# Cyan4973/FiniteStateEntropy

Measured on AMD Instinct MI355X. Metric: MB/s encode+decode per GPU on 32KB probagen blocks; bit-exact vs CPU ref, higher is better.
Workload: dtype u8; 1 GPU; probagen Proba14, 100000 x 32KB blocks per GPU, FSE encode+decode (one-shot calls at the reference's default limits: tableLog 11, decode maxLog 12), bit-exact check; blocks_per_gpu=100000, block_bytes=32768, codec=fse, parity=fse: roundtrip-all-blocks

## Files before the change

finitestateentropy_amd/csrc/fse_tables.hip:

```cpp
#include "internal.h"

#include "wave_glue.h"
#include "ncount_reader.h"
#include "fse_wave_build.h"

template <u32 MAXC>
DEV void fse_wave_build_ctable(const WaveBuildLds& w, const int nn[4], u32 maxSV, u32 tl, u32* img, u32 lane)
{
    u16* const cumAll = w.cumP;
    *(uint2*)(w.nrm + 4 * lane) = make_uint2(((u32)nn[0] & 0xFFFFu) | ((u32)nn[1] << 16), ((u32)nn[2] & 0xFFFFu) | ((u32)nn[3] << 16));
    __syncthreads();
    const u32 ts = 1u << tl;
    u16* const stateTable = (u16*)(img + 1);
    u32* const tt = img + 1 + (ts >> 1);
    {
        u32 eff[4], laneSum = 0;
#pragma unroll
        for (int i = 0; i < 4; ++i) { eff[i] = nn[i] == -1 ? 1u : (u32)nn[i]; laneSum += eff[i]; }
        u32 total;
        u32 run = wb_scan_excl(laneSum, lane, &total);
#pragma unroll
        for (int i = 0; i < 4; ++i) {
            const u32 s = 4 * lane + i;
            cumAll[s] = (u16)run;
            if (s <= maxSV) {
                if (nn[i] == 0) { tt[2 * s] = 0; tt[2 * s + 1] = ((tl + 1) << 16) - ts; }
                else if (nn[i] == -1 || nn[i] == 1) { tt[2 * s] = run - 1u; tt[2 * s + 1] = (tl << 16) - ts; }
                else {
                    const u32 maxBitsOut = tl - hibit32((u32)nn[i] - 1);
                    tt[2 * s] = run - (u32)nn[i];
                    tt[2 * s + 1] = (maxBitsOut << 16) - ((u32)nn[i] << maxBitsOut);
                }
            }
            run += eff[i];
        }
        if (lane == 0) img[0] = tl | (maxSV << 16);
    }
    __syncthreads();
    wave_spread_rank<MAXC>(w, maxSV, tl, lane, [&](u32 s) { return (u32)cumAll[s]; },
                     [&](u32 u, u32 s, u32 r, u32 first) { (void)s; stateTable[first + r] = (u16)(ts + u); });
}

template <u32 MAXC>
__global__ __launch_bounds__(64) void k_fse_cprep(FseCPrepArgs a, u32 capTs)
{
    extern __shared__ __attribute__((aligned(16))) u8 wbLds[];
    const size_t b = blockIdx.x;
    const u32 lane = threadIdx.x;
    const size_t n = view_size(a.src, b);
    FseMeta m; m.state = 0; m.hdrSize = 0; m.tableLog = 0; m.maxSV = 0; m.pace = 0;
    const size_t top = a.histResults[b];
    size_t result = 0; bool go = false;
    if (n <= 1) result = 0;
    else if (is_err(top)) result = top;
    else if (top == n) result = 1;
    else if (top == 1 || top < (n >> 7)) result = 0;
    else go = true;
    const WaveBuildLds w = wave_build_carve(wbLds, capTs, true);
    u32* const hdrImg = w.cnt;
    u32 maxSV = 0, tl = 0;
    int nn[4] = { 0, 0, 0, 0 };
    if (go) {
        maxSV = a.maxSVs[b];
        tl = wg_optimal_tablelog(a.tableLogReq, n, maxSV, 2);
        if ((1u << tl) > 64u * MAXC || (1u << tl) > capTs) { result = FERR(tableLog_tooLarge); go = false; }
    }
    if (go) {
        const uint4 cv = ((const uint4*)(a.counts + b * 256))[lane];
        const u32 c[4] = { cv.x, cv.y, cv.z, cv.w };
        for (u32 i = lane; i < 136; i += 64) hdrImg[i] = 0;
        const size_t e = wg_normalize<64>(nn, c, (u64)n, maxSV, tl, lane);
        if (is_err(e)) { result = e; go = false; }
    }
    __syncthreads();
    if (go) {
        const size_t h = wg_write_ncount<64>(hdrImg, a.dstCapacity, nn, maxSV, tl, lane);
        if (is_err(h)) { result = h; go = false; }
        else m.hdrSize = (u32)h;
    }
    __syncthreads();
    if (!go) { if (lane == 0) { a.meta[b] = m; a.results[b] = result; } return; }
    {   u8* const dst = a.dst + b * a.dstStride;
        const u8* const hb = (const u8*)hdrImg;
        for (u32 i = lane; i < m.hdrSize; i += 64) dst[i] = hb[i];
    }
    int top1 = nn[0] > nn[1] ? nn[0] : nn[1]; top1 = nn[2] > top1 ? nn[2] : top1; top1 = nn[3] > top1 ? nn[3] : top1;
    top1 = wave_max_i32(top1);
    m.state = ((u32)top1 * 64u > (63u << tl) || n < FSE_ENC_WAVE_MIN) ? FSE_ENC_LANE : FSE_ENC_PAR;
    {
        u32 present = (nn[0] != 0) + (nn[1] != 0) + (nn[2] != 0) + (nn[3] != 0);
        present = wg_sum<64>(present);
        const u32 mix = (1u << tl) / (present ? present : 1u);
        m.pace = mix < 64u ? 0u : mix < 128u ? 1u : mix < 256u ? 2u : 3u;
    }
    m.tableLog = tl; m.maxSV = maxSV;
    if (lane == 0) a.meta[b] = m;
    fse_wave_build_ctable<MAXC>(w, nn, maxSV, tl, a.ctables + b * a.ctStrideU32, lane);
}

__global__ __launch_bounds__(64) void k_fse_dparse(FseDPrepArgs a)
{
    __shared__ __attribute__((aligned(16))) u32 stage[NCS_WORDS];
    const size_t b0 = (size_t)blockIdx.x * 64, b = b0 + threadIdx.x;
    const u32 lane = threadIdx.x;
    const bool have = b < a.nBlocks;
    const u8* const in = have ? view_ptr(a.csrc, b) : nullptr;
    const size_t cSize = have ? view_size(a.csrc, b) : 0;
    bool done = false;
    if (have && a.rawRle) { const size_t orig = a.origSizes ? a.origSizes[b] : a.uniformOrig; done = cSize == orig || cSize == 1; }
    const u32 staged = ncount_stage(stage, in, cSize, lane, have && !done);
    {   uint4* const rows = (uint4*)(a.norms + b0 * 256);
        const u32 nRows = a.nBlocks - b0 < 64 ? (u32)(a.nBlocks - b0) : 64u;
        for (u32 i = lane; i < nRows * 32u; i += 64) rows[i] = make_uint4(0, 0, 0, 0);
    }
    __syncthreads();
    int cls = -1;
    if (have) {
        FseMeta m; m.state = 0; m.hdrSize = 0; m.tableLog = 0; m.maxSV = 0; m.pace = 0; m.pace = 0;
        size_t result = 0;
        if (!done) do {
            u32 tl = 0, maxSV = 255;
            s16* const norm = a.norms + b * 256;
            const size_t h = ncount_read_staged(norm, &maxSV, &tl, stage + lane, staged, in, cSize);
            if (is_err(h)) { result = h; break; }
            if (tl > a.maxLog) { result = FERR(tableLog_tooLarge); break; }
            cls = FSE_DCLS_REV11;
            if (tl > FSE_DEC_FAST_MAXLOG) {
                int top = 0;
                for (u32 i = 0; i <= maxSV >> 3; ++i) {
                    const uint4 v = ((const uint4*)norm)[i];
                    const u32 q[4] = { v.x, v.y, v.z, v.w };
#pragma unroll
                    for (int k = 0; k < 4; ++k) { const int lo = (s16)(q[k] & 0xFFFFu), hi = (s16)(q[k] >> 16); top = lo > top ? lo : top; top = hi > top ? hi : top; }
                }
                cls = 2 * top > (1 << tl) ? FSE_DCLS_PLAIN : FSE_DCLS_REV12;
            }
            m.state = 1u | ((u32)cls << 2); m.hdrSize = (u32)h; m.tableLog = tl; m.maxSV = maxSV;
        } while (0);
        a.meta[b] = m;
        if (m.state == 0 && !done) a.results[b] = result;
    }
    if (cls >= 0) { const size_t bin = view_size(a.csrc, b) >> FSE_DBIN_LOG; cls = cls * FSE_DBINS + (int)(bin < FSE_DBINS - 1 ? bin : FSE_DBINS - 1); }
    const unsigned long long below = (1ull << lane) - 1ull;
    unsigned long long todo = __ballot(cls >= 0);
    while (todo) {
        const int leader = __builtin_ctzll(todo);
        const int c = __shfl(cls, leader, WAVE);
        const unsigned long long mask = __ballot(cls == c);
        u32 base = 0;
        if ((int)lane == leader) {
            base = atomicAdd(&a.counts[c], (u32)__builtin_popcountll(mask));
            atomicAdd(&a.counts[FSE_DCLS_COUNT + c / FSE_DBINS], (u32)__builtin_popcountll(mask));
        }
        base = (u32)__shfl((int)base, leader, WAVE);
        if (cls == c) a.lists[(size_t)c * a.nBlocks + base + (u32)__builtin_popcountll(mask & below)] = (u32)b;
        todo &= ~mask;
    }
}

template <u32 MAXC>
__global__ __launch_bounds__(64) void k_fse_dbuild(FseDPrepArgs a, u32 capTs, int firstList, int nLists, u32 ldsCapTs)
{
    extern __shared__ __attribute__((aligned(16))) u8 wbLds[];
    {   u32 total = 0;
        for (int k = firstList / (int)FSE_DBINS; k < (firstList + nLists) / (int)FSE_DBINS; ++k) total += a.counts[FSE_DCLS_COUNT + k];
        if (blockIdx.x >= total) return;
    }
    constexpr int MAXL = 2 * FSE_DBINS;
    static_assert(FSE_DBINS % 4 == 0, "the list lengths are read as 16-byte vectors");
    uint4 cv[MAXL / 4];
#pragma unroll
    for (int i = 0; i < MAXL / 4; ++i) cv[i] = 4 * i < nLists ? ((const uint4*)(a.counts + firstList))[i] : make_uint4(0, 0, 0, 0);
    u32 idx = blockIdx.x;
    int c = firstList + nLists;
    {   u32 before = 0; bool found = false;
#pragma unroll
        for (int i = 0; i < MAXL; ++i) {
            const uint4 v = cv[i >> 2];
            const u32 n = (i & 3) == 0 ? v.x : (i & 3) == 1 ? v.y : (i & 3) == 2 ? v.z : v.w;
            const bool here = !found & (i < nLists) & (idx < before + n);
            c = here ? firstList + i : c; idx = here ? idx - before : idx;
            found |= here;
            before += n;
        }
    }
    if (c == firstList + nLists) return;
    const size_t b = a.lists[(size_t)c * a.nBlocks + idx];
    const u32 lane = threadIdx.x;
    const FseMeta m = a.meta[b];
    if (m.state == 0) return;
    const u32 tl = m.tableLog, ts = 1u << tl;
    if (ts > ldsCapTs || ts > 64u * MAXC) {
        if (lane == 0) { a.meta[b].state = 0; a.results[b] = FERR(tableLog_tooLarge); }
        return;
    }
    const WaveBuildLds w = wave_build_carve(wbLds, ldsCapTs, false);
    *(uint2*)(w.nrm + 4 * lane) = *(const uint2*)(a.norms + b * 256 + 4 * lane);
    __syncthreads();
    const bool rev = ((m.state >> 2) & 3u) != FSE_DCLS_PLAIN;
    u16* const A = a.atab + b * capTs;
    u8* const S = a.symtab + b * capTs;
    const bool fast = wave_spread_rank<MAXC>(w, m.maxSV, tl, lane, [&](u32 s) { return (u32)(int)w.nrm[s]; }, [&](u32 u, u32 s, u32 r, u32 nrm) {
        const int n = (int)nrm;
        const u32 next = (n > 0 ? (u32)n : 1u) + r;
        const u32 nb = tl - hibit32(next);
        const u32 ns = (next << nb) - ts;
        const u32 x = rev ? __brev(u) >> (32u - tl) : u;
        A[x] = rev ? (u16)(nb | ((__brev(ns) >> (32u - tl)) << 5)) : (u16)((ns & 0xFFFu) | (nb << 12));
        S[x] = (u8)s;
    });
    if (lane == 0) a.meta[b].state = m.state | (fast ? 2u : 0u);
}

__global__ __launch_bounds__(256) void k_fse_export_dtable(FseDPrepArgs a, u32 capTs, u32* dtables, size_t dtStrideU32)
{
    const size_t b = blockIdx.x;
    const FseMeta m = a.meta[b];
    if (m.state == 0) return;
    const u32 tl = m.tableLog, ts = 1u << tl;
    const bool rev = ((m.state >> 2) & 3u) != FSE_DCLS_PLAIN;
    const u16* const A = a.atab + b * capTs;
    const u8* const S = a.symtab + b * capTs;
    u32* const dt = dtables + b * dtStrideU32;
    if (threadIdx.x == 0) dt[0] = tl | ((m.state & 2u) ? 1u << 16 : 0u);
    for (u32 x = threadIdx.x; x < ts; x += blockDim.x) {
        const u32 i = rev ? __brev(x) >> (32u - tl) : x;
        const u32 c = A[i];
        const u32 nb = rev ? (c & 31u) : (c >> 12);
        const u32 ns = rev ? __brev(c >> 5) >> (32u - tl) : (c & 0xFFFu);
        dt[1 + x] = ns | ((u32)S[i] << 16) | (nb << 24);
    }
}
hipError_t launch_fse_export_dtables(const FseDPrepArgs& a, u32* dtables, size_t dtStrideU32, hipStream_t s)
{
    if (a.nBlocks == 0) return hipSuccess;
    hipLaunchKernelGGL(k_fse_export_dtable, dim3((unsigned)a.nBlocks), dim3(256), 0, s, a, 1u << a.maxLog, dtables, dtStrideU32);
    return hipGetLastError();
}

DEV size_t fse_norm_load_checked(int nn[4], const s16* nb, u32 maxSV, u32 tl, u32 maxTl, u32 lane)
{
    if (maxSV > 255u) return FERR(maxSymbolValue_tooLarge);
    if (tl > maxTl) return FERR(tableLog_tooLarge);
    if (tl == 0 || tl == 1 || tl == 3) return FERR(GENERIC);
    u32 cells = 0; bool bad = false;
#pragma unroll
    for (int i = 0; i < 4; ++i) {
        nn[i] = 4 * lane + i <= maxSV ? (int)nb[4 * lane + i] : 0;
        bad |= nn[i] < -1;
        cells += nn[i] == -1 ? 1u : nn[i] > 0 ? (u32)nn[i] : 0u;
    }
    cells = wg_sum<64>(cells);
    return (wg_any<64>(bad, lane) || cells != (1u << tl)) ? FERR(GENERIC) : 0;
}
template <u32 MAXC>
__global__ __launch_bounds__(64) void k_fse_ctable_from_norm(const s16* norms, size_t normStride, const u32* maxSVs, u32 tl, u32* ctables, size_t ctStrideU32,
                                                            size_t* results, u32 capTs)
{
    extern __shared__ __attribute__((aligned(16))) u8 wbLds[];
    const size_t b = blockIdx.x;
    const u32 lane = threadIdx.x;
    const u32 maxSV = maxSVs[b];
    int nn[4] = { 0, 0, 0, 0 };
    static_assert(MAXC == 32 || MAXC == 64, "64 * MAXC cells = a table of tableLog 11 or 12");
    const size_t r = fse_norm_load_checked(nn, norms + b * normStride, maxSV, tl, MAXC == 32 ? 11u : FSE_MAX_TL, lane);
    if (lane == 0) results[b] = r;
    if (is_err(r)) return;
    fse_wave_build_ctable<MAXC>(wave_build_carve(wbLds, capTs, true), nn, maxSV, tl, ctables + b * ctStrideU32, lane);
}
hipError_t launch_fse_ctable_from_norm(const s16* norms, size_t normStride, const u32* maxSVs, u32 tl, u32* ctables, size_t ctStrideU32, size_t* results,
                                       size_t nBlocks, hipStream_t s)
{
    if (nBlocks == 0) return hipSuccess;
    const u32 capTs = 1u << (tl >= 1 && tl <= FSE_MAX_TL ? tl : FSE_MAX_TL);
    if (wb_small(capTs))
        hipLaunchKernelGGL(k_fse_ctable_from_norm<32>, dim3((unsigned)nBlocks), dim3(64), wave_build_lds_bytes(capTs, true), s, norms, normStride, maxSVs, tl, ctables,
                           ctStrideU32, results, capTs);
    else
        hipLaunchKernelGGL(k_fse_ctable_from_norm<64>, dim3((unsigned)nBlocks), dim3(64), wave_build_lds_bytes(capTs, true), s, norms, normStride, maxSVs, tl, ctables,
                           ctStrideU32, results, capTs);
    return hipGetLastError();
}

static void launch_fse_dbuild_lists(const FseDPrepArgs& a, u32 capTs, int firstList, int nLists, u32 ldsCapTs, hipStream_t s)
{
    if (wb_small(ldsCapTs))
        hipLaunchKernelGGL(k_fse_dbuild<32>, dim3((unsigned)a.nBlocks), dim3(64), wave_build_lds_bytes(ldsCapTs, false), s, a, capTs, firstList, nLists, ldsCapTs);
    else
        hipLaunchKernelGGL(k_fse_dbuild<64>, dim3((unsigned)a.nBlocks), dim3(64), wave_build_lds_bytes(ldsCapTs, false), s, a, capTs, firstList, nLists, ldsCapTs);
}
static void launch_fse_dbuilds(const FseDPrepArgs& a, hipStream_t s)
{
    const u32 capTs = 1u << a.maxLog;
    const u32 capA = a.maxLog < FSE_DEC_FAST_MAXLOG ? capTs : (1u << FSE_DEC_FAST_MAXLOG);
    launch_fse_dbuild_lists(a, capTs, (int)FSE_DCLS_REV11 * FSE_DBINS, (int)FSE_DBINS, capA, s);
    if (a.maxLog > FSE_DEC_FAST_MAXLOG) launch_fse_dbuild_lists(a, capTs, (int)FSE_DCLS_REV12 * FSE_DBINS, 2 * (int)FSE_DBINS, capTs, s);
}

__global__ __launch_bounds__(64) void k_fse_dmeta_from_norm(FseDPrepArgs a, const s16* norms, size_t normStride, const u32* maxSVs, u32 tl)
{
    const size_t b = blockIdx.x;
    const u32 lane = threadIdx.x;
    const u32 maxSV = maxSVs[b];
    int nn[4] = { 0, 0, 0, 0 };
    const size_t r = fse_norm_load_checked(nn, norms + b * normStride, maxSV, tl, a.maxLog, lane);
    FseMeta m; m.state = 0; m.hdrSize = 0; m.tableLog = tl; m.maxSV = maxSV; m.pace = 0;
    if (!is_err(r)) {
        *(uint2*)(a.norms + b * 256 + 4 * lane) = make_uint2(((u32)nn[0] & 0xFFFFu) | ((u32)nn[1] << 16), ((u32)nn[2] & 0xFFFFu) | ((u32)nn[3] << 16));
        int top = nn[0] > nn[1] ? nn[0] : nn[1]; top = nn[2] > top ? nn[2] : top; top = nn[3] > top ? nn[3] : top;
        top = wave_max_i32(top);
        const u32 cls = tl <= FSE_DEC_FAST_MAXLOG ? (u32)FSE_DCLS_REV11 : 2 * top > (1 << tl) ? (u32)FSE_DCLS_PLAIN : (u32)FSE_DCLS_REV12;
        m.state = 1u | (cls << 2);
        if (lane == 0) {
            const u32 at = atomicAdd(&a.counts[cls * FSE_DBINS], 1u);
            atomicAdd(&a.counts[FSE_DCLS_COUNT + cls], 1u);
            a.lists[(size_t)cls * FSE_DBINS * a.nBlocks + at] = (u32)b;
        }
    }
    if (lane == 0) { a.meta[b] = m; if (is_err(r)) a.results[b] = r; }
}
hipError_t launch_fse_dprep_from_norm(const FseDPrepArgs& a, const s16* norms, size_t normStride, const u32* maxSVs, u32 tl, hipStream_t s)
{
    if (a.nBlocks == 0) return hipSuccess;
    hipError_t e = launch_zero_u32(a.counts, FSE_DCLS_COUNT + FSE_DCLS_KINDS, s);
    if (e != hipSuccess) return e;
    hipLaunchKernelGGL(k_fse_dmeta_from_norm, dim3((unsigned)a.nBlocks), dim3(64), 0, s, a, norms, normStride, maxSVs, tl);
    launch_fse_dbuilds(a, s);
    return hipGetLastError();
}

#ifdef FSE_WB_TIMING
extern "C" __attribute__((visibility("default"))) int FSEHIP_debug_wbTiming(unsigned long long* host) { return (int)hipMemcpyFromSymbol(host, HIP_SYMBOL(g_wbTiming), sizeof(g_wbTiming)); }
#endif
__global__ __launch_bounds__(64) void k_fse_glue_normalize(s16* norms, size_t normStride, u32 tlReq, const u32* counts, size_t countStride,
                                                          const size_t* totals, const u32* maxSVs, size_t* results)
{
    const size_t b = blockIdx.x;
    const u32 lane = threadIdx.x;
    const u32 maxSV = maxSVs[b] > 255u ? 255u : maxSVs[b];
    const u32* const cb = counts + b * countStride;
    u32 c[4];
#pragma unroll
    for (int i = 0; i < 4; ++i) c[i] = 4 * lane + i <= maxSV ? cb[4 * lane + i] : 0u;
    int nn[4] = { 0, 0, 0, 0 };
    const u32 tl = tlReq ? tlReq : FSE_DEF_TL;
    const u64 total = (u64)totals[b];
    size_t r = total ? wg_normalize<64>(nn, c, total, maxSV, tl, lane) : FERR(GENERIC);
    if (!is_err(r)) r = tl;
    s16* const nb = norms + b * normStride;
#pragma unroll
    for (int i = 0; i < 4; ++i) if (4 * lane + i <= maxSV && !is_err(r)) nb[4 * lane + i] = (s16)nn[i];
    if (lane == 0) results[b] = r;
}

__global__ __launch_bounds__(64) void k_fse_glue_write_ncount(u8* headers, size_t headerStride, size_t headerCapacity, const s16* norms, size_t normStride,
                                                             const u32* maxSVs, u32 tl, size_t* results)
{
    __shared__ u32 img[136];
    const size_t b = blockIdx.x;
    const u32 lane = threadIdx.x;
    const u32 maxSV = maxSVs[b];
    size_t r;
    if (tl > FSE_MAX_TL) r = FERR(tableLog_tooLarge);
    else if (tl < FSE_MIN_TL || maxSV > 255u) r = FERR(GENERIC);
    else {
        const s16* const nb = norms + b * normStride;
        int nn[4];
#pragma unroll
        for (int i = 0; i < 4; ++i) nn[i] = 4 * lane + i <= maxSV ? (int)nb[4 * lane + i] : 0;
        for (u32 i = lane; i < 136; i += 64) img[i] = 0;
        __syncthreads();
        r = wg_write_ncount<64>(img, headerCapacity, nn, maxSV, tl, lane);
        __syncthreads();
        if (!is_err(r)) {
            u8* const dst = headers + b * headerStride;
            const u8* const hb = (const u8*)img;
            for (u32 i = lane; i < (u32)r; i += 64) dst[i] = hb[i];
        }
    }
    if (lane == 0) results[b] = r;
}

__global__ __launch_bounds__(64) void k_fse_glue_read_ncount(s16* norms, size_t normStride, u32* maxSVs, u32* tableLogs, BlockView headers, size_t nBlocks, size_t* results)
{
    const size_t b = (size_t)blockIdx.x * 64 + threadIdx.x;
    if (b >= nBlocks) return;
    u32 maxSV = maxSVs[b], tl = 0;
    size_t r;
    if ((size_t)maxSV >= normStride) r = FERR(maxSymbolValue_tooLarge);
    else r = ncount_read<1>(norms + b * normStride, &maxSV, &tl, view_ptr(headers, b), view_size(headers, b));
    if (!is_err(r)) { maxSVs[b] = maxSV; tableLogs[b] = tl; }
    results[b] = r;
}

hipError_t launch_fse_glue_normalize(s16* norms, size_t normStride, u32 tl, const u32* counts, size_t countStride, const size_t* totals, const u32* maxSVs,
                                     size_t* results, size_t nBlocks, hipStream_t s)
{
    if (nBlocks == 0) return hipSuccess;
    hipLaunchKernelGGL(k_fse_glue_normalize, dim3((unsigned)nBlocks), dim3(64), 0, s, norms, normStride, tl, counts, countStride, totals, maxSVs, results);
    return hipGetLastError();
}
hipError_t launch_fse_glue_write_ncount(u8* headers, size_t headerStride, size_t headerCapacity, const s16* norms, size_t normStride, const u32* maxSVs, u32 tl,
                                        size_t* results, size_t nBlocks, hipStream_t s)
{
    if (nBlocks == 0) return hipSuccess;
    hipLaunchKernelGGL(k_fse_glue_write_ncount, dim3((unsigned)nBlocks), dim3(64), 0, s, headers, headerStride, headerCapacity, norms, normStride, maxSVs, tl, results);
    return hipGetLastError();
}
hipError_t launch_fse_glue_read_ncount(s16* norms, size_t normStride, u32* maxSVs, u32* tableLogs, const BlockView& headers, size_t* results, size_t nBlocks, hipStream_t s)
{
    if (nBlocks == 0) return hipSuccess;
    hipLaunchKernelGGL(k_fse_glue_read_ncount, dim3((unsigned)((nBlocks + 63) / 64)), dim3(64), 0, s, norms, normStride, maxSVs, tableLogs, headers, nBlocks, results);
    return hipGetLastError();
}

hipError_t launch_fse_cprep(const FseCPrepArgs& a, hipStream_t s)
{
    if (a.nBlocks == 0) return hipSuccess;
    const u32 capTs = 1u << a.maxTl;
    const size_t ldsBytes = wave_build_lds_bytes(capTs, true);
    probe_before(PK_FSE_CPREP, s);
    if (wb_small(capTs)) hipLaunchKernelGGL(k_fse_cprep<32>, dim3((unsigned)a.nBlocks), dim3(64), ldsBytes, s, a, capTs);
    else hipLaunchKernelGGL(k_fse_cprep<64>, dim3((unsigned)a.nBlocks), dim3(64), ldsBytes, s, a, capTs);
    probe_after(PK_FSE_CPREP, s);
    return hipGetLastError();
}
hipError_t launch_fse_dprep(const FseDPrepArgs& a, hipStream_t s)
{
    if (a.nBlocks == 0) return hipSuccess;
    hipError_t e = launch_zero_u32(a.counts, FSE_DCLS_COUNT + FSE_DCLS_KINDS, s);
    if (e != hipSuccess) return e;
    probe_before(PK_FSE_DPREP, s);
    hipLaunchKernelGGL(k_fse_dparse, dim3((unsigned)((a.nBlocks + 63) / 64)), dim3(64), 0, s, a);
    launch_fse_dbuilds(a, s);
    probe_after(PK_FSE_DPREP, s);
    return hipGetLastError();
}
```

finitestateentropy_amd/csrc/fse_wave_build.h:

```cpp
#pragma once
#include "dev_common.h"

#define WB_MAXSYM 256
#ifndef WB_WIN
#define WB_WIN 64u
#endif
#define WB_TSTEP(ts) (((ts) >> 1) + ((ts) >> 3) + 3)

#ifdef FSE_WB_TIMING
__device__ unsigned long long g_wbTiming[4096 * 8];
#define WBT(k) TT[k] = __builtin_readcyclecounter();
#else
#define WBT(k)
#endif
struct WaveBuildLds {
    s16* nrm;
    u16* cumP;
    u8*  symP;
    u8*  symTab;
    u8*  marks;
    u32* cnt;
    u16* coarse;
};
__host__ __device__ inline u32 wb_si(u32 u) { return u + ((u >> 5) << 2); }
#ifndef WB_EXTRA_LDS
#define WB_EXTRA_LDS 0u
#endif
__host__ __device__ inline size_t wb_up16(size_t n) { return (n + 15) & ~(size_t)15; }
__host__ __device__ inline size_t wb_part_a(u32 capTs) { const size_t m = wb_si(capTs); return wb_up16(m > WB_WIN * 64 ? m : WB_WIN * 64); }
__host__ __device__ inline size_t wb_part_b(u32 capTs) { const size_t t = wb_si(capTs); return wb_up16(t > WB_WIN * 32 ? t : WB_WIN * 32); }
__host__ __device__ inline size_t wave_build_lds_bytes(u32 capTs, bool withCum) { return wb_part_a(capTs) + wb_part_b(capTs) + 512 + 256 + (withCum ? 528 : 0) + WB_EXTRA_LDS; }
DEV WaveBuildLds wave_build_carve(u8* base, u32 capTs, bool withCum)
{
    WaveBuildLds w;
    w.cnt = (u32*)base; w.marks = base; base += wb_part_a(capTs);
    w.coarse = (u16*)base; w.symTab = base; base += wb_part_b(capTs);
    w.nrm = (s16*)base; base += 512;
    w.symP = base; base += 256;
    w.cumP = withCum ? (u16*)base : nullptr;
    return w;
}
__host__ __device__ inline bool wb_small(u32 capTs) { return capTs <= 2048u; }

DEV u32 wb_bytesum(u32 v) { return __builtin_amdgcn_sad_u8(v, 0u, 0u); }
DEV u32 wb_scan_excl(u32 v, u32 lane, u32* total)
{
#if FSEHIP_DPP_SCANS
    const u32 incl = group_scan_incl<64, ScanAdd>(v, lane);
    *total = group_last<64>(incl, lane);
#else
    u32 incl = v;
#pragma unroll
    for (int off = 1; off < 64; off <<= 1) { const u32 o = (u32)__shfl_up((int)incl, off, WAVE); if ((int)lane >= off) incl += o; }
    *total = (u32)__shfl((int)incl, 63, WAVE);
#endif
    return incl - v;
}

DEV void wb_opaque(u32& v) { asm volatile("" : "+v"(v)); }
#define WB_MAXC ((1u << FSEHIP_FSE_MAX_TABLELOG) >> 6)

template <u32 MAXC, class Payload, class Emit>
DEV bool wave_spread_rank(const WaveBuildLds& w, u32 maxSV, u32 tl, u32 lane, Payload&& payload, Emit&& emit)
{
#ifdef FSE_WB_TIMING
    unsigned long long TT[8];
#endif
    WBT(0)
    const u32 ts = 1u << tl, mask = ts - 1, step = WB_TSTEP(ts);
    const u32 C = ts >= 64 ? ts >> 6 : 1;
    const bool act = lane * C < ts;
    const u32 m0 = lane * C;
    static_assert(MAXC % 8 == 0 && MAXC <= WB_MAXC, "cells per lane: whole groups of eight, at most the largest table's");
    u8* const marks = w.marks;
    int n[4];
    {   const uint2 raw = *(const uint2*)(w.nrm + 4 * lane);
        n[0] = (s16)(raw.x & 0xFFFFu); n[1] = (s16)(raw.x >> 16); n[2] = (s16)(raw.y & 0xFFFFu); n[3] = (s16)(raw.y >> 16);
    }
    u32 lanePos = 0, laneLow = 0, laneAny = 0; bool big = false;
#pragma unroll
    for (int i = 0; i < 4; ++i) {
        if (4 * lane + i > maxSV) n[i] = 0;
        lanePos += n[i] > 0 ? (u32)n[i] : 0u; laneLow += n[i] == -1; laneAny += n[i] != 0;
        big |= n[i] >= (int)(ts >> 1);
    }
    u32 totals;
    const u32 base3 = wb_scan_excl(lanePos | (laneLow << 13) | (laneAny << 22), lane, &totals);
    u32 posBase = base3 & 0x1FFFu, lowBase = (base3 >> 13) & 0x1FFu, anyBase = base3 >> 22;
    const u32 nLow = (totals >> 13) & 0x1FFu, nAny = totals >> 22;
    const int high = (int)ts - 1 - (int)nLow;
    if (act) { if (C >= 4) for (u32 i = 0; i < C; i += 4) *(u32*)(marks + wb_si(m0 + i)) = 0; else for (u32 i = 0; i < C; ++i) marks[wb_si(m0 + i)] = 0; }
    __syncthreads();
    WBT(1)
#pragma unroll
    for (int i = 0; i < 4; ++i) {
        if (n[i] != 0) w.symP[anyBase++] = (u8)(4 * lane + i);
        if (n[i] > 0) { marks[wb_si(posBase)] = (u8)(4 * lane + i); posBase += (u32)n[i]; }
        else if (n[i] == -1) { w.symTab[wb_si(ts - 1 - lowBase)] = (u8)(4 * lane + i); ++lowBase; }
    }
    u32 nv = 0;
    if (act) { u32 u = (m0 * step) & mask; for (u32 i = 0; i < C; ++i) { nv += (int)u <= high; u = (u + step) & mask; } }
    u32 totalKept;
    const u32 k0 = wb_scan_excl(nv, lane, &totalKept);
    __syncthreads();
    WBT(2)
    u32 localMax = 0;
    for (u32 i = 0; i < nv; i += 8) {
        u32 v[8];
#pragma unroll
        for (u32 j = 0; j < 8; ++j) { const u32 idx = k0 + i + j; v[j] = marks[wb_si(idx < ts ? idx : ts - 1)]; }
#pragma unroll
        for (u32 j = 0; j < 8; ++j) if (i + j < nv) localMax = v[j] > localMax ? v[j] : localMax;
    }
    u32 run = localMax;
#if FSEHIP_DPP_SCANS
    run = group_scan_incl<64, ScanMax>(run, lane);
    run = dpp_mov<0x138, 0xF, true>(0u, run);
#else
#pragma unroll
    for (int off = 1; off < 64; off <<= 1) { const u32 o = (u32)__shfl_up((int)run, off, WAVE); if ((int)lane >= off) run = o > run ? o : run; }
    run = (u32)__shfl_up((int)run, 1, WAVE);
    if (lane == 0) run = 0;
#endif
    if (act && nv) {
        u32 u = (m0 * step) & mask, k = k0;
        u32 i = 0;
        for (; i + 8 <= C; i += 8) {
            u32 uu[8], v[8]; bool keep[8];
#pragma unroll
            for (u32 j = 0; j < 8; ++j) {
                uu[j] = u; keep[j] = (int)u <= high;
                v[j] = marks[wb_si(k < ts ? k : ts - 1)];
                k += keep[j]; u = (u + step) & mask;
            }
#pragma unroll
            for (u32 j = 0; j < 8; ++j) if (keep[j]) { run = v[j] > run ? v[j] : run; w.symTab[wb_si(uu[j])] = (u8)run; }
        }
        for (; i < C; ++i) {
            if ((int)u <= high) { const u32 v = marks[wb_si(k)]; ++k; run = v > run ? v : run; w.symTab[wb_si(u)] = (u8)run; }
            u = (u + step) & mask;
        }
    }
    __syncthreads();
    WBT(3)

    const u32 nj = C < 8 ? C : 8;
    u32 sym[MAXC / 4], lr[MAXC / 4];
#pragma unroll
    for (u32 q = 0; q < MAXC / 4; ++q) { sym[q] = 0; lr[q] = 0; }
    if (act) {
        if (C >= 8) {
#pragma unroll
            for (u32 g = 0; g < MAXC / 8; ++g)
                if (8 * g < C) {
                    const u32* const syp = (const u32*)(w.symTab + wb_si(m0 + 8 * g));
                    sym[2 * g] = syp[0]; sym[2 * g + 1] = syp[1];
                }
        } else {
#pragma unroll
            for (u32 j = 0; j < 4; ++j) if (j < C) sym[0] |= (u32)w.symTab[wb_si(m0 + j)] << (8 * j);
        }
    }
    const u32 sh8 = 8 * (lane & 3u), grp = lane >> 2;
    const u32 belowMask = (1u << sh8) - 1u;
    const bool single = maxSV < WB_WIN;
    for (u32 base = 0; base <= maxSV; base += WB_WIN) {
        {   const u32 rows = (maxSV + 1 - base) < WB_WIN ? (maxSV + 1 - base) : WB_WIN;
            for (u32 i = 4 * lane; i < rows * 16; i += 256) *(uint4*)(w.cnt + i) = make_uint4(0, 0, 0, 0);
        }
        __syncthreads();
        if (act) {
#pragma unroll
            for (u32 g = 0; g < MAXC / 8; ++g) {
                if (8 * g >= C) break;
                wb_opaque(sym[2 * g]); wb_opaque(sym[2 * g + 1]);
                u32 old[8]; bool in[8];
#pragma unroll
                for (u32 j = 0; j < 8; ++j) {
                    const u32 s = ((sym[2 * g + (j >> 2)] >> (8 * (j & 3))) & 0xFFu) - base;
                    in[j] = j < nj && (single || s < WB_WIN);
                    old[j] = 0;
                    if (in[j]) old[j] = atomicAdd(&w.cnt[s * 16 + grp], 1u << sh8);
                }
#pragma unroll
                for (u32 h = 0; h < 2; ++h) {
                    u32 r = lr[2 * g + h];
#pragma unroll
                    for (u32 k = 0; k < 4; ++k) {
                        const u32 j = 4 * h + k;
                        if (in[j]) r = (r & ~(0xFFu << (8 * k))) | (((old[j] >> sh8) & 0xFFu) << (8 * k));
                    }
                    lr[2 * g + h] = r;
                }
            }
        }
        __syncthreads();
        WBT(4)
        for (u32 j = lane; j < nAny; j += 64) {
            const u32 s = (u32)w.symP[j] - base;
            if (!single && s >= WB_WIN) continue;
            const uint4* const row = (const uint4*)(w.cnt + s * 16);
            const uint4 c0 = row[0], c1 = row[1], c2 = row[2], c3 = row[3];
            u32 r[16];
            u32 acc = 0;
#define WB_ACC(k, v) r[k] = acc; acc += wb_bytesum(v);
            WB_ACC(0, c0.x) WB_ACC(1, c0.y) WB_ACC(2, c0.z) WB_ACC(3, c0.w) WB_ACC(4, c1.x) WB_ACC(5, c1.y) WB_ACC(6, c1.z) WB_ACC(7, c1.w)
            WB_ACC(8, c2.x) WB_ACC(9, c2.y) WB_ACC(10, c2.z) WB_ACC(11, c2.w) WB_ACC(12, c3.x) WB_ACC(13, c3.y) WB_ACC(14, c3.z) WB_ACC(15, c3.w)
#undef WB_ACC
            uint4* const out = (uint4*)(w.coarse + s * 16);
            out[0] = make_uint4(r[0] | (r[1] << 16), r[2] | (r[3] << 16), r[4] | (r[5] << 16), r[6] | (r[7] << 16));
            out[1] = make_uint4(r[8] | (r[9] << 16), r[10] | (r[11] << 16), r[12] | (r[13] << 16), r[14] | (r[15] << 16));
        }
        __syncthreads();
        WBT(5)
        if (act) {
#pragma unroll
            for (u32 g = 0; g < MAXC / 8; ++g) {
                if (8 * g >= C) break;
                wb_opaque(sym[2 * g]); wb_opaque(sym[2 * g + 1]);
                u32 mg = m0 + 8 * g; wb_opaque(mg);
                u32 sf[8], co[8], cn[8], pl[8]; bool in[8];
#pragma unroll
                for (u32 j = 0; j < 8; ++j) {
                    sf[j] = (sym[2 * g + (j >> 2)] >> (8 * (j & 3))) & 0xFFu;
                    const u32 sw = sf[j] - base;
                    in[j] = j < nj && (single || sw < WB_WIN);
                    const u32 row = in[j] ? sw : 0u;
                    co[j] = w.coarse[row * 16 + grp]; cn[j] = w.cnt[row * 16 + grp]; pl[j] = payload(sf[j]);
                }
#pragma unroll
                for (u32 j = 0; j < 8; ++j) {
                    const u32 local = (lr[2 * g + (j >> 2)] >> (8 * (j & 3))) & 0xFFu;
                    if (in[j]) emit(mg + j, sf[j], local + co[j] + wb_bytesum(cn[j] & belowMask), pl[j]);
                }
            }
        }
        __syncthreads();
    }
    WBT(6)
#ifdef FSE_WB_TIMING
    if (lane == 0 && blockIdx.x < 4096) for (int q = 0; q < 6; ++q) g_wbTiming[8 * blockIdx.x + q] = TT[q + 1] - TT[q];
#endif
    return !__any(big);
}
```

Measured before the change: 207,300 MiB/s of uncompressed data through encode+decode (whole job).

## Build FSE state table image in LDS and copy out coalesced

For small tables (tableLog up to 11), the compression-table build now assembles the state table as a u16 image in otherwise-dead LDS and copies it to global memory with coalesced 32-bit stores. Previously each symbol's state was scattered straight to global memory with 16-bit stores. Symbol transform entries are now written as vectorized 2- or 4-word stores, and the header copy uses word-wide unaligned stores instead of byte stores. The cost is an extra LDS pass, 16-bit packed ranks in registers, and a new guard that rejects carve sizes too small for the image.

```diff
diff --git a/finitestateentropy_amd/csrc/fse_tables.hip b/finitestateentropy_amd/csrc/fse_tables.hip
--- a/finitestateentropy_amd/csrc/fse_tables.hip
+++ b/finitestateentropy_amd/csrc/fse_tables.hip
@@ -4,6 +4,18 @@
 #include "ncount_reader.h"
 #include "fse_wave_build.h"
 
+#ifndef FSE_CT_IMAGE_MAXC
+#define FSE_CT_IMAGE_MAXC 32u
+#endif
+typedef u32 u32x4_a4 __attribute__((ext_vector_type(4), aligned(4)));
+typedef u32 u32x2_a4 __attribute__((ext_vector_type(2), aligned(4)));
+typedef u32 u32_a1 __attribute__((aligned(1)));
+DEV void wave_copy_out_bytes(u8* dst, const u32* image, u32 n, u32 lane)
+{
+    for (u32 i = lane; i < n >> 2; i += 64) *(u32_a1*)(dst + 4 * i) = image[i];
+    const u32 done = n & ~3u;
+    if (lane < n - done) dst[done + lane] = ((const u8*)image)[done + lane];
+}
 template <u32 MAXC>
 DEV void fse_wave_build_ctable(const WaveBuildLds& w, const int nn[4], u32 maxSV, u32 tl, u32* img, u32 lane)
 {
@@ -19,26 +31,37 @@
         for (int i = 0; i < 4; ++i) { eff[i] = nn[i] == -1 ? 1u : (u32)nn[i]; laneSum += eff[i]; }
         u32 total;
         u32 run = wb_scan_excl(laneSum, lane, &total);
+        u32 e[8];
 #pragma unroll
         for (int i = 0; i < 4; ++i) {
-            const u32 s = 4 * lane + i;
-            cumAll[s] = (u16)run;
-            if (s <= maxSV) {
-                if (nn[i] == 0) { tt[2 * s] = 0; tt[2 * s + 1] = ((tl + 1) << 16) - ts; }
-                else if (nn[i] == -1 || nn[i] == 1) { tt[2 * s] = run - 1u; tt[2 * s + 1] = (tl << 16) - ts; }
-                else {
-                    const u32 maxBitsOut = tl - hibit32((u32)nn[i] - 1);
-                    tt[2 * s] = run - (u32)nn[i];
-                    tt[2 * s + 1] = (maxBitsOut << 16) - ((u32)nn[i] << maxBitsOut);
-                }
+            cumAll[4 * lane + i] = (u16)run;
+            if (nn[i] == 0) { e[2 * i] = 0; e[2 * i + 1] = ((tl + 1) << 16) - ts; }
+            else if (nn[i] == -1 || nn[i] == 1) { e[2 * i] = run - 1u; e[2 * i + 1] = (tl << 16) - ts; }
+            else {
+                const u32 maxBitsOut = tl - hibit32((u32)nn[i] - 1);
+                e[2 * i] = run - (u32)nn[i];
+                e[2 * i + 1] = (maxBitsOut << 16) - ((u32)nn[i] << maxBitsOut);
             }
             run += eff[i];
         }
+#pragma unroll
+        for (int h = 0; h < 2; ++h) {
+            const u32 s = 4 * lane + 2 * h;
+            if (s + 1 <= maxSV) { u32x4_a4 v; v.x = e[4 * h]; v.y = e[4 * h + 1]; v.z = e[4 * h + 2]; v.w = e[4 * h + 3]; *(u32x4_a4*)(tt + 2 * s) = v; }
+            else if (s <= maxSV) { u32x2_a4 v; v.x = e[4 * h]; v.y = e[4 * h + 1]; *(u32x2_a4*)(tt + 2 * s) = v; }
+        }
         if (lane == 0) img[0] = tl | (maxSV << 16);
     }
     __syncthreads();
-    wave_spread_rank<MAXC>(w, maxSV, tl, lane, [&](u32 s) { return (u32)cumAll[s]; },
-                     [&](u32 u, u32 s, u32 r, u32 first) { (void)s; stateTable[first + r] = (u16)(ts + u); });
+    if constexpr (MAXC <= FSE_CT_IMAGE_MAXC) {
+        wave_spread_image<MAXC>(w, maxSV, tl, lane, [&](u32 s) { return (u32)cumAll[s]; });
+        const u32* const image = w.cnt;
+        u32* const st = (u32*)stateTable;
+#pragma unroll 4
+        for (u32 i = lane; i < ts >> 1; i += 64) st[i] = image[i];
+    } else
+        wave_spread_rank<MAXC>(w, maxSV, tl, lane, [&](u32 s) { return (u32)cumAll[s]; },
+                         [&](u32 u, u32 s, u32 r, u32 first) { (void)s; stateTable[first + r] = (u16)(ts + u); });
 }
 
 template <u32 MAXC>
@@ -47,6 +70,10 @@
     extern __shared__ __attribute__((aligned(16))) u8 wbLds[];
     const size_t b = blockIdx.x;
     const u32 lane = threadIdx.x;
+#ifdef FSE_WB_TIMING
+    unsigned long long TT[8];
+#endif
+    WBT(0)
     const size_t n = view_size(a.src, b);
     FseMeta m; m.state = 0; m.hdrSize = 0; m.tableLog = 0; m.maxSV = 0; m.pace = 0;
     const size_t top = a.histResults[b];
@@ -73,6 +100,7 @@
         if (is_err(e)) { result = e; go = false; }
     }
     __syncthreads();
+    WBT(1)
     if (go) {
         const size_t h = wg_write_ncount<64>(hdrImg, a.dstCapacity, nn, maxSV, tl, lane);
         if (is_err(h)) { result = h; go = false; }
@@ -80,10 +108,8 @@
     }
     __syncthreads();
     if (!go) { if (lane == 0) { a.meta[b] = m; a.results[b] = result; } return; }
-    {   u8* const dst = a.dst + b * a.dstStride;
-        const u8* const hb = (const u8*)hdrImg;
-        for (u32 i = lane; i < m.hdrSize; i += 64) dst[i] = hb[i];
-    }
+    wave_copy_out_bytes(a.dst + b * a.dstStride, hdrImg, m.hdrSize, lane);
+    WBT(2)
     int top1 = nn[0] > nn[1] ? nn[0] : nn[1]; top1 = nn[2] > top1 ? nn[2] : top1; top1 = nn[3] > top1 ? nn[3] : top1;
     top1 = wave_max_i32(top1);
     m.state = ((u32)top1 * 64u > (63u << tl) || n < FSE_ENC_WAVE_MIN) ? FSE_ENC_LANE : FSE_ENC_PAR;
@@ -96,6 +122,12 @@
     m.tableLog = tl; m.maxSV = maxSV;
     if (lane == 0) a.meta[b] = m;
     fse_wave_build_ctable<MAXC>(w, nn, maxSV, tl, a.ctables + b * a.ctStrideU32, lane);
+#ifdef FSE_WB_TIMING
+    WBT(3)
+    asm volatile("s_waitcnt vmcnt(0)" ::: "memory");
+    WBT(4)
+    if (lane == 0 && blockIdx.x < 4096) for (int q = 0; q < 4; ++q) g_wbTiming[WBT_STRIDE * blockIdx.x + 8 + q] = TT[q + 1] - TT[q];
+#endif
 }
 
 __global__ __launch_bounds__(64) void k_fse_dparse(FseDPrepArgs a)
@@ -273,6 +305,7 @@
 {
     if (nBlocks == 0) return hipSuccess;
     const u32 capTs = 1u << (tl >= 1 && tl <= FSE_MAX_TL ? tl : FSE_MAX_TL);
+    if (!wb_image_fits(capTs)) return hipErrorInvalidValue;
     if (wb_small(capTs))
         hipLaunchKernelGGL(k_fse_ctable_from_norm<32>, dim3((unsigned)nBlocks), dim3(64), wave_build_lds_bytes(capTs, true), s, norms, normStride, maxSVs, tl, ctables,
                            ctStrideU32, results, capTs);
@@ -419,6 +452,7 @@
     if (a.nBlocks == 0) return hipSuccess;
     const u32 capTs = 1u << a.maxTl;
     const size_t ldsBytes = wave_build_lds_bytes(capTs, true);
+    if (!wb_image_fits(capTs)) return hipErrorInvalidValue;
     probe_before(PK_FSE_CPREP, s);
     if (wb_small(capTs)) hipLaunchKernelGGL(k_fse_cprep<32>, dim3((unsigned)a.nBlocks), dim3(64), ldsBytes, s, a, capTs);
     else hipLaunchKernelGGL(k_fse_cprep<64>, dim3((unsigned)a.nBlocks), dim3(64), ldsBytes, s, a, capTs);
diff --git a/finitestateentropy_amd/csrc/fse_wave_build.h b/finitestateentropy_amd/csrc/fse_wave_build.h
--- a/finitestateentropy_amd/csrc/fse_wave_build.h
+++ b/finitestateentropy_amd/csrc/fse_wave_build.h
@@ -8,7 +8,8 @@
 #define WB_TSTEP(ts) (((ts) >> 1) + ((ts) >> 3) + 3)
 
 #ifdef FSE_WB_TIMING
-__device__ unsigned long long g_wbTiming[4096 * 8];
+#define WBT_STRIDE 16
+__device__ unsigned long long g_wbTiming[4096 * WBT_STRIDE];
 #define WBT(k) TT[k] = __builtin_readcyclecounter();
 #else
 #define WBT(k)
@@ -22,13 +23,13 @@
     u32* cnt;
     u16* coarse;
 };
-__host__ __device__ inline u32 wb_si(u32 u) { return u + ((u >> 5) << 2); }
+__host__ __device__ constexpr u32 wb_si(u32 u) { return u + ((u >> 5) << 2); }
 #ifndef WB_EXTRA_LDS
 #define WB_EXTRA_LDS 0u
 #endif
-__host__ __device__ inline size_t wb_up16(size_t n) { return (n + 15) & ~(size_t)15; }
-__host__ __device__ inline size_t wb_part_a(u32 capTs) { const size_t m = wb_si(capTs); return wb_up16(m > WB_WIN * 64 ? m : WB_WIN * 64); }
-__host__ __device__ inline size_t wb_part_b(u32 capTs) { const size_t t = wb_si(capTs); return wb_up16(t > WB_WIN * 32 ? t : WB_WIN * 32); }
+__host__ __device__ constexpr size_t wb_up16(size_t n) { return (n + 15) & ~(size_t)15; }
+__host__ __device__ constexpr size_t wb_part_a(u32 capTs) { const size_t m = wb_si(capTs); return wb_up16(m > WB_WIN * 64 ? m : WB_WIN * 64); }
+__host__ __device__ constexpr size_t wb_part_b(u32 capTs) { const size_t t = wb_si(capTs); return wb_up16(t > WB_WIN * 32 ? t : WB_WIN * 32); }
 __host__ __device__ inline size_t wave_build_lds_bytes(u32 capTs, bool withCum) { return wb_part_a(capTs) + wb_part_b(capTs) + 512 + 256 + (withCum ? 528 : 0) + WB_EXTRA_LDS; }
 DEV WaveBuildLds wave_build_carve(u8* base, u32 capTs, bool withCum)
 {
@@ -41,6 +42,8 @@
     return w;
 }
 __host__ __device__ inline bool wb_small(u32 capTs) { return capTs <= 2048u; }
+__host__ __device__ constexpr bool wb_image_fits(u32 capTs) { return (size_t)2 * capTs <= (capTs <= 2048u ? wb_part_a(capTs) : wb_part_a(capTs) + wb_part_b(capTs)); }
+static_assert(wb_image_fits(2048u) && wb_image_fits(1u << FSEHIP_FSE_MAX_TABLELOG), "the state-table image of the largest tables must fit in the dead parts of the carve");
 
 DEV u32 wb_bytesum(u32 v) { return __builtin_amdgcn_sad_u8(v, 0u, 0u); }
 DEV u32 wb_scan_excl(u32 v, u32 lane, u32* total)
@@ -60,11 +63,11 @@
 DEV void wb_opaque(u32& v) { asm volatile("" : "+v"(v)); }
 #define WB_MAXC ((1u << FSEHIP_FSE_MAX_TABLELOG) >> 6)
 
-template <u32 MAXC, class Payload, class Emit>
-DEV bool wave_spread_rank(const WaveBuildLds& w, u32 maxSV, u32 tl, u32 lane, Payload&& payload, Emit&& emit)
+template <u32 MAXC, bool IMAGE, class Payload, class Emit>
+DEV bool wave_spread_rank_core(const WaveBuildLds& w, u32 maxSV, u32 tl, u32 lane, Payload&& payload, Emit&& emit)
 {
 #ifdef FSE_WB_TIMING
-    unsigned long long TT[8];
+    unsigned long long TT[10];
 #endif
     WBT(0)
     const u32 ts = 1u << tl, mask = ts - 1, step = WB_TSTEP(ts);
@@ -145,9 +148,10 @@
     WBT(3)
 
     const u32 nj = C < 8 ? C : 8;
-    u32 sym[MAXC / 4], lr[MAXC / 4];
-#pragma unroll
-    for (u32 q = 0; q < MAXC / 4; ++q) { sym[q] = 0; lr[q] = 0; }
+    constexpr u32 FB = IMAGE ? 16u : 8u, FM = (1u << FB) - 1u, FPR = 32u / FB;
+    u32 sym[MAXC / 4], lr[MAXC / FPR];
+#pragma unroll
+    for (u32 q = 0; q < MAXC / FPR; ++q) { if (q < MAXC / 4) sym[q] = 0; lr[q] = 0; }
     if (act) {
         if (C >= 8) {
 #pragma unroll
@@ -183,14 +187,14 @@
                     if (in[j]) old[j] = atomicAdd(&w.cnt[s * 16 + grp], 1u << sh8);
                 }
 #pragma unroll
-                for (u32 h = 0; h < 2; ++h) {
-                    u32 r = lr[2 * g + h];
-#pragma unroll
-                    for (u32 k = 0; k < 4; ++k) {
-                        const u32 j = 4 * h + k;
-                        if (in[j]) r = (r & ~(0xFFu << (8 * k))) | (((old[j] >> sh8) & 0xFFu) << (8 * k));
+                for (u32 h = 0; h < 8 / FPR; ++h) {
+                    u32 r = lr[8 / FPR * g + h];
+#pragma unroll
+                    for (u32 k = 0; k < FPR; ++k) {
+                        const u32 j = FPR * h + k;
+                        if (in[j]) r = (r & ~(FM << (FB * k))) | (((old[j] >> sh8) & 0xFFu) << (FB * k));
                     }
-                    lr[2 * g + h] = r;
+                    lr[8 / FPR * g + h] = r;
                 }
             }
         }
@@ -230,16 +234,42 @@
                 }
 #pragma unroll
                 for (u32 j = 0; j < 8; ++j) {
-                    const u32 local = (lr[2 * g + (j >> 2)] >> (8 * (j & 3))) & 0xFFu;
-                    if (in[j]) emit(mg + j, sf[j], local + co[j] + wb_bytesum(cn[j] & belowMask), pl[j]);
+                    const u32 q = (8 * g + j) / FPR, fs = FB * (j % FPR);
+                    const u32 local = (lr[q] >> fs) & FM;
+                    if constexpr (IMAGE) { if (in[j]) lr[q] = (lr[q] & ~(FM << fs)) | ((pl[j] + local + co[j] + wb_bytesum(cn[j] & belowMask)) << fs); }
+                    else if (in[j]) emit(mg + j, sf[j], local + co[j] + wb_bytesum(cn[j] & belowMask), pl[j]);
                 }
             }
         }
         __syncthreads();
     }
     WBT(6)
+    if constexpr (IMAGE) {
+        u16* const image = (u16*)w.cnt;
+        if (act) {
+#pragma unroll
+            for (u32 g = 0; g < MAXC / 8; ++g) {
+                if (8 * g >= C) break;
+#pragma unroll
+                for (u32 j = 0; j < 8; ++j)
+                    if (j < nj) image[(lr[(8 * g + j) / FPR] >> (FB * (j % FPR))) & mask] = (u16)(ts + m0 + 8 * g + j);
+            }
+        }
+        __syncthreads();
+    }
+    WBT(7)
 #ifdef FSE_WB_TIMING
-    if (lane == 0 && blockIdx.x < 4096) for (int q = 0; q < 6; ++q) g_wbTiming[8 * blockIdx.x + q] = TT[q + 1] - TT[q];
+    if (lane == 0 && blockIdx.x < 4096) for (int q = 0; q < 7; ++q) g_wbTiming[WBT_STRIDE * blockIdx.x + q] = TT[q + 1] - TT[q];
 #endif
     return !__any(big);
 }
+template <u32 MAXC, class Payload, class Emit>
+DEV bool wave_spread_rank(const WaveBuildLds& w, u32 maxSV, u32 tl, u32 lane, Payload&& payload, Emit&& emit)
+{
+    return wave_spread_rank_core<MAXC, false>(w, maxSV, tl, lane, payload, emit);
+}
+template <u32 MAXC, class First>
+DEV void wave_spread_image(const WaveBuildLds& w, u32 maxSV, u32 tl, u32 lane, First&& first)
+{
+    wave_spread_rank_core<MAXC, true>(w, maxSV, tl, lane, first, [](u32, u32, u32, u32) {});
+}
```

Measured after the change: 208,900 MiB/s of uncompressed data through encode+decode (whole job) (median of 6 runs). Within noise of the previous version (+0.8%).
